# kvas7andy/unreal

Measured on AMD Instinct MI355X. Metric: env-steps/sec (whole node), UNREAL maze 84x84, higher is better.
Workload: dtype f32 (fp16x2-split MFMA operands, fp32 accumulate)

## Files before the change

### unreal_amd/csrc/pc.hip

```cpp
#include "common.h"

namespace {

constexpr int HP_LD = 36, HP_ROWS = 84;
constexpr int NPLP = 2;
constexpr int WD_ELEMS = 4 * 4 * 2 * 4 * 16 * 4;
constexpr int HP_V = (C2_POS * 8 + 255) / 256;
constexpr int DD_V = (PC_CELLS * 8 / 4 + 255) / 256;

struct PcFwdArgs {
  int N, A;
  const float* hp;
  const float* hp_absmax;
  const float* Wv; const float* bv; const float* Wa; const float* ba;
  float* qmax;
  const int* action;
  const float* target;
  const int* mask;
  float lambda, grad_scale;
  float* d_dec;
  float* ddec_absmax;
  float* loss;
};

// ... 11 lines not shown
    int id = gtid + 256 * c;
    r[c] = s4[id < C2_POS * 8 ? id : gtid];
  }
}

__device__ __forceinline__ void hp_store(float* hp, int gtid, const f32x4 (&r)[HP_V]) {
#pragma unroll
  for (int c = 0; c < HP_V; ++c) {
    int id = gtid + 256 * c;
    if (id < C2_POS * 8) *reinterpret_cast<f32x4*>(hp + (id >> 3) * HP_LD + (id & 7) * 4) = r[c];
  }
}

typedef _Float16 fh8p __attribute__((ext_vector_type(8)));
typedef _Float16 fh2p __attribute__((ext_vector_type(2)));
typedef float f32x2p __attribute__((ext_vector_type(2)));
typedef unsigned int u32x2p __attribute__((ext_vector_type(2)));

constexpr int HPP_ROW = 80;
constexpr int HPP_PLANE = HP_ROWS * HPP_ROW;
constexpr int WDP_ROW = 80;
constexpr int WDP_PLANE = 4 * 32 * WDP_ROW;

__device__ __forceinline__ void split4p(const f32x4& v, float scale, u32x2p (&pl)[NPLP]) {
  const f32x2p x01 = (f32x2p){v[0], v[1]} * scale, x23 = (f32x2p){v[2], v[3]} * scale;
  const fh2p h01 = __builtin_convertvector(x01, fh2p), h23 = __builtin_convertvector(x23, fh2p);
  const fh2p l01 = __builtin_convertvector(x01 - __builtin_convertvector(h01, f32x2p), fh2p);
  const fh2p l23 = __builtin_convertvector(x23 - __builtin_convertvector(h23, f32x2p), fh2p);
  pl[0] = (u32x2p){__builtin_bit_cast(unsigned int, h01), __builtin_bit_cast(unsigned int, h23)};
  pl[1] = (u32x2p){__builtin_bit_cast(unsigned int, l01), __builtin_bit_cast(unsigned int, l23)};
}

__device__ __forceinline__ void hp_store_planes(unsigned char* hpp, int gtid, const f32x4 (&r)[HP_V], float scale) {
#pragma unroll
  for (int c = 0; c < HP_V; ++c) {
    const int id = gtid + 256 * c;
    if (id < C2_POS * 8) {
      u32x2p pl[NPLP];
      split4p(r[c], scale, pl);
      pl[0][0] = keep_positive_visible(pl[0][0], r[c][0], r[c][1]);
      pl[0][1] = keep_positive_visible(pl[0][1], r[c][2], r[c][3]);
#pragma unroll
      for (int t = 0; t < NPLP; ++t) *reinterpret_cast<u32x2p*>(hpp + t * HPP_PLANE + (id >> 3) * HPP_ROW + (id & 7) * 8) = pl[t];
    }
  }
}

#define PC_MFMA(a, b, c) __builtin_amdgcn_mfma_f32_16x16x32_f16((a), (b), (c), 0, 0, 0)
#define PC_SPLIT_MMA(A, B, C)        \
  do {                               \
    C = PC_MFMA(A[1], B[0], C);      \
    C = PC_MFMA(A[0], B[1], C);      \
    C = PC_MFMA(A[0], B[0], C);      \
  } while (0)

__device__ __forceinline__ float pc_weight_max(const float* __restrict__ Wv, const float* __restrict__ Wa, int A, float* red) {
  if (threadIdx.x == 0) *red = 0.f;
  __syncthreads();
  float m = 0.f;
  for (int e = threadIdx.x; e < 512; e += 256) m = fmaxf(m, fabsf(Wv[e]));
  for (int e = threadIdx.x; e < 512 * A; e += 256) m = fmaxf(m, fabsf(Wa[e]));
  m = wave_max(m);
  if ((threadIdx.x & 63) == 0) atomicMax(reinterpret_cast<unsigned int*>(red), __float_as_uint(m));
  __syncthreads();
  return *red;
}

__device__ __forceinline__ void pc_fwd_weight_planes(const float* __restrict__ Wv, const float* __restrict__ Wa, int A,
                                                     unsigned char* wdp, float S_W) {
  const int CO = 1 + A;
  for (int e = threadIdx.x; e < 4 * 32 * 8; e += 256) {
    const int c4 = e & 7, n = (e >> 3) & 31, dd = e >> 8;
    f32x4 v = {0.f, 0.f, 0.f, 0.f};
    if (n < 4 * CO) {
      const int par = n / CO, co = n - par * CO;
      const int ky = (par >> 1) + 2 * (dd >> 1), kx = (par & 1) + 2 * (dd & 1);
#pragma unroll
      for (int k = 0; k < 4; ++k) v[k] = deconv_w(Wv, Wa, A, ky, kx, co, 4 * c4 + k);
    }
    u32x2p pl[NPLP];
    split4p(v, S_W, pl);
#pragma unroll
    for (int t = 0; t < NPLP; ++t) *reinterpret_cast<u32x2p*>(wdp + t * WDP_PLANE + (dd * 32 + n) * WDP_ROW + c4 * 8) = pl[t];
  }
}

__device__ __forceinline__ void pc_zero_hp_pad_rows(unsigned char* hpp) {
  for (int e = threadIdx.x; e < NPLP * 3 * HPP_ROW / 4; e += 256) {
    const int t = e / (3 * HPP_ROW / 4), w = e % (3 * HPP_ROW / 4);
    reinterpret_cast<uint32_t*>(hpp + t * HPP_PLANE + C2_POS * HPP_ROW)[w] = 0u;
  }
}

template <int COT> struct FwdLds {
  static constexpr int DS = COT | 1;
  static constexpr int DEC = NPLP * HPP_PLANE, DOUT = DEC + PC_CELLS * DS * 4, W = DOUT + PC_CELLS * COT * 4,
                       BYTES = W + NPLP * WDP_PLANE;
  static constexpr int WGS = 3 * BYTES <= 160 * 1024 ? 3 : 2;
};

template <bool TWO_NT, int DS>
__device__ __forceinline__ void deconv_packed(const unsigned char* hpp, const unsigned char* wdp, float* dec, int mt0, int i,
                                              int q, int CO, const float (&bias)[2], float unscale) {
  constexpr int NTL = TWO_NT ? 2 : 1;
  const int ntiles = (mt0 + 4 < 7) ? 2 : 1;
  f32x4 acc[2][NTL];
  int a[2], b[2];
#pragma unroll
  for (int t = 0; t < 2; ++t) {
#pragma unroll
    for (int nt = 0; nt < NTL; ++nt) acc[t][nt] = (f32x4){0.f, 0.f, 0.f, 0.f};
    const int m = min((mt0 + 4 * t) * 16 + i, 99);
    a[t] = m / 10;
    b[t] = m % 10;
  }
#pragma unroll
  for (int dd = 0; dd < 4; ++dd) {
    const int da = dd >> 1, db = dd & 1;
    fh8p bw[NTL][NPLP];
#pragma unroll
    for (int nt = 0; nt < NTL; ++nt)
#pragma unroll
      for (int pl = 0; pl < NPLP; ++pl)
        bw[nt][pl] = *reinterpret_cast<const fh8p*>(wdp + pl * WDP_PLANE + ((dd * 32 + nt * 16 + i)) * WDP_ROW + 16 * q);
#pragma unroll
    for (int t = 0; t < 2; ++t) {
      if (t < ntiles) {
        const int y = a[t] - da, x = b[t] - db;
        const int row = (y >= 0 && y < 9 && x >= 0 && x < 9) ? y * 9 + x : C2_POS;
        fh8p av[NPLP];
#pragma unroll
        for (int pl = 0; pl < NPLP; ++pl)
          av[pl] = *reinterpret_cast<const fh8p*>(hpp + pl * HPP_PLANE + row * HPP_ROW + 16 * q);
#pragma unroll
        for (int nt = 0; nt < NTL; ++nt) PC_SPLIT_MMA(av, bw[nt], acc[t][nt]);
      }
    }
  }
#pragma unroll
  for (int nt = 0; nt < NTL; ++nt) {
    const int n = nt * 16 + i;
    if (n < 4 * CO) {
      const int par = n / CO, co = n - par * CO;
#pragma unroll
      for (int t = 0; t < 2; ++t)
        if (t < ntiles) {
#pragma unroll
          for (int r = 0; r < 4; ++r) {
            const int m = (mt0 + 4 * t) * 16 + 4 * q + r;
            if (m < 100)
              dec[((2 * (m / 10) + (par >> 1)) * 20 + 2 * (m % 10) + (par & 1)) * DS + co] = acc[t][nt][r] * unscale + bias[nt];
          }
        }
    }
  }
}

template <int COT>
__global__ __launch_bounds__(256, FwdLds<COT>::WGS) void pc_deconv_fwd_kernel(PcFwdArgs p) {
  typedef FwdLds<COT> L;
  constexpr int DS = L::DS;
  __shared__ __attribute__((aligned(16))) unsigned char smem[L::BYTES];
  __shared__ float s_red;
  const int gtid = threadIdx.x;
  const int lane = threadIdx.x & 63, gw = gtid >> 6;
  const int i = lane & 15, q = lane >> 4;
  unsigned char* hpp = smem;
  float* dec = reinterpret_cast<float*>(smem + L::DEC);
  float* dout = reinterpret_cast<float*>(smem + L::DOUT);
  unsigned char* wdp = smem + L::W;
  const int A = p.A, CO = 1 + p.A;

  const float S_W = pow2_scale(pc_weight_max(p.Wv, p.Wa, A, &s_red));
  const float S_HP = pow2_scale(*p.hp_absmax);
  const float unscale = pow2_inv(S_HP) * pow2_inv(S_W);

  pc_fwd_weight_planes(p.Wv, p.Wa, A, wdp, S_W);
  pc_zero_hp_pad_rows(hpp);
  float bias[2];
#pragma unroll
  for (int nt = 0; nt < 2; ++nt) {
    const int n = nt * 16 + i;
    const int co = n % CO;
    bias[nt] = (n < 4 * CO) ? (co == 0 ? p.bv[0] : p.ba[co - 1]) : 0.f;
  }
  const bool two_nt = 4 * CO > 16;
  float loss_acc = 0.f, dd_max = 0.f;

  const int stride = gridDim.x;
  f32x4 pre[HP_V];
  {
    const int n0 = blockIdx.x;
    if (n0 < p.N) {
      hp_load(p.hp + (size_t)n0 * F2_DIM, gtid, pre);
      hp_store_planes(hpp, gtid, pre, S_HP);
    }
  }
  int prev = -1;
  for (int base = blockIdx.x; base < p.N; base += stride) {
    const int n = base;
    const bool valid = n < p.N;
// ... 67 lines not shown
      if (p.ddec_absmax) absmax_commit(p.ddec_absmax, fmaxf(fmaxf(wmx[0], wmx[1]), fmaxf(wmx[2], wmx[3])));
    }
  }
}

struct PcBwdArgs {
  int N, A;
  const float* hp;
  const float* hp_absmax;
  const float* d_dec;
  const float* ddec_absmax;
  const float* Wv; const float* Wa;
  float* d_hp;
  float* dWv; float* dbv; float* dWa; float* dba;
  float* dhp_absmax;
};

typedef short s16x4p __attribute__((ext_vector_type(4)));
typedef short s16x8p __attribute__((ext_vector_type(8)));
constexpr int DDP_ROW = 16;
constexpr int DDP_PLANE = (PC_CELLS + 4) * DDP_ROW;
constexpr int WBP_PLANE = 4 * 32 * WDP_ROW;
constexpr int BWD_GRP_BYTES = NPLP * HPP_PLANE + NPLP * DDP_PLANE + F2_DIM * 4;

__device__ __forceinline__ fh8p tr_pair_p(const unsigned char* a0, const unsigned char* a1) {
  typedef s16x4p __attribute__((address_space(3))) * lds_p;
  const s16x4p lo = __builtin_amdgcn_ds_read_tr16_b64_v4i16((lds_p)(a0));
  const s16x4p hi = __builtin_amdgcn_ds_read_tr16_b64_v4i16((lds_p)(a1));
  const s16x8p v = __builtin_shufflevector(lo, hi, 0, 1, 2, 3, 4, 5, 6, 7);
  return __builtin_bit_cast(fh8p, v);
}

__device__ __forceinline__ void split1p(float x, float scale, unsigned short (&t)[NPLP]) {
  x *= scale;
  const _Float16 h = (_Float16)x;
  const _Float16 l = (_Float16)(x - (float)h);
  t[0] = __builtin_bit_cast(unsigned short, h);
  t[1] = __builtin_bit_cast(unsigned short, l);
}

__device__ __forceinline__ void pc_bwd_weight_planes(const float* __restrict__ Wv, const float* __restrict__ Wa, int A,
                                                     unsigned char* wbp, float S_W) {
  for (int e = threadIdx.x; e < 4 * 32 * 32; e += 256) {
    const int k = e & 31, ci = (e >> 5) & 31, ky = e >> 10;
    const int kx = k >> 3, co = k & 7;
    float v = 0.f;
    if (co == 0) v = Wv[(ky * 4 + kx) * 32 + ci];
    else if (co <= A) v = Wa[((ky * 4 + kx) * A + (co - 1)) * 32 + ci];
    unsigned short t[NPLP];
    split1p(v, S_W, t);
#pragma unroll
    for (int pl = 0; pl < NPLP; ++pl)
      reinterpret_cast<unsigned short*>(wbp + pl * WBP_PLANE + (ky * 32 + ci) * WDP_ROW)[k] = t[pl];
  }
}

__device__ __forceinline__ void pc_stage_dd(unsigned char* ddp, int gtid, const float (&dd)[2][8], float S_DD, float (&adbk)[8]) {
#pragma unroll
  for (int h = 0; h < 2; ++h) {
    const int pos = gtid + 256 * h;
    if (pos < PC_CELLS) {
      u32x2p lo[NPLP], hi[NPLP];
      split4p((f32x4){dd[h][0], dd[h][1], dd[h][2], dd[h][3]}, S_DD, lo);
      split4p((f32x4){dd[h][4], dd[h][5], dd[h][6], dd[h][7]}, S_DD, hi);
#pragma unroll
      for (int pl = 0; pl < NPLP; ++pl) {
        typedef unsigned int u32x4p __attribute__((ext_vector_type(4)));
        *reinterpret_cast<u32x4p*>(ddp + pl * DDP_PLANE + pos * DDP_ROW) = (u32x4p){lo[pl][0], lo[pl][1], hi[pl][0], hi[pl][1]};
      }
#pragma unroll
      for (int k = 0; k < 8; ++k) adbk[k] += dd[h][k];
    }
  }
}

__device__ __forceinline__ void pc_dgrad_frame(const unsigned char* hpp, const unsigned char* ddp, const unsigned char* wbp,
                                               float* dhs, int gw, int i, int q, float un_dgrad) {
  const int nt = gw & 1;
  f32x4 acc[3];
  int abase[3];
#pragma unroll
  for (int jj = 0; jj < 3; ++jj) {
    acc[jj] = (f32x4){0.f, 0.f, 0.f, 0.f};
    const int pos = min(((gw >> 1) + 2 * jj) * 16 + i, C2_POS - 1);
    abase[jj] = ((2 * (pos / 9)) * 20 + 2 * (pos % 9) + q) * DDP_ROW;
  }
#pragma unroll
  for (int ky = 0; ky < 4; ++ky) {
    fh8p bw[NPLP];
#pragma unroll
    for (int pl = 0; pl < NPLP; ++pl)
      bw[pl] = *reinterpret_cast<const fh8p*>(wbp + pl * WBP_PLANE + (ky * 32 + nt * 16 + i) * WDP_ROW + 16 * q);
#pragma unroll
    for (int jj = 0; jj < 3; ++jj) {
      fh8p av[NPLP];
#pragma unroll
      for (int pl = 0; pl < NPLP; ++pl)
        av[pl] = *reinterpret_cast<const fh8p*>(ddp + pl * DDP_PLANE + abase[jj] + ky * 20 * DDP_ROW);
      PC_SPLIT_MMA(av, bw, acc[jj]);
    }
  }
#pragma unroll
  for (int jj = 0; jj < 3; ++jj)
#pragma unroll
    for (int r = 0; r < 4; ++r) {
      const int pos = ((gw >> 1) + 2 * jj) * 16 + 4 * q + r;
      if (pos < C2_POS) {
        const int ci = nt * 16 + i;
        const unsigned short h0 = reinterpret_cast<const unsigned short*>(hpp + pos * HPP_ROW)[ci];
        dhs[pos * 32 + ci] = (h0 != 0 && !(h0 & 0x8000)) ? acc[jj][r] * un_dgrad : 0.f;
      }
    }
}

__device__ __forceinline__ void pc_wgrad_frame(const unsigned char* hpp, const unsigned char* ddp, int gw, int i, int q,
                                               f32x4 (&aw)[2][2]) {
  const int qq = i >> 2, pp = i & 3;
#pragma unroll 1
  for (int ks = 0; ks < 3; ++ks) {
    const int p0 = 32 * ks + 8 * q + qq, p1 = p0 + 4;
    const unsigned char* b0 = hpp + min(p0, C2_POS) * HPP_ROW + 8 * pp;
    const unsigned char* b1 = hpp + min(p1, C2_POS) * HPP_ROW + 8 * pp;
    fh8p bf[2][NPLP];
#pragma unroll
    for (int t = 0; t < 2; ++t)
#pragma unroll
      for (int pl = 0; pl < NPLP; ++pl) bf[t][pl] = tr_pair_p(b0 + pl * HPP_PLANE + 32 * t, b1 + pl * HPP_PLANE + 32 * t);
    const int r0 = p0 < C2_POS ? (2 * (p0 / 9) + gw) * 20 + 2 * (p0 % 9) : PC_CELLS;
    const int r1 = p1 < C2_POS ? (2 * (p1 / 9) + gw) * 20 + 2 * (p1 % 9) : PC_CELLS;
#pragma unroll
    for (int kxh = 0; kxh < 2; ++kxh) {
      fh8p af[NPLP];
#pragma unroll
      for (int pl = 0; pl < NPLP; ++pl)
        af[pl] = tr_pair_p(ddp + pl * DDP_PLANE + (r0 + 2 * kxh) * DDP_ROW + 8 * pp,
                           ddp + pl * DDP_PLANE + (r1 + 2 * kxh) * DDP_ROW + 8 * pp);
      PC_SPLIT_MMA(af, bf[0], aw[kxh][0]);
      PC_SPLIT_MMA(af, bf[1], aw[kxh][1]);
    }
  }
}

__device__ __forceinline__ float pc_drain_dhp(const float* dhs, float* __restrict__ dst_frame, int gtid, float dhp_max) {
  f32x4* dst = reinterpret_cast<f32x4*>(dst_frame);
  for (int id = gtid; id < F2_DIM / 4; id += 256) {
    const f32x4 v = reinterpret_cast<const f32x4*>(dhs)[id];
    dst[id] = v;
    dhp_max = fmaxf(fmaxf(dhp_max, fmaxf(fabsf(v[0]), fabsf(v[1]))), fmaxf(fabsf(v[2]), fabsf(v[3])));
  }
  return dhp_max;
}

__device__ __forceinline__ void pc_commit_grads(const f32x4 (&aw)[2][2], float un_wgrad, const float (&adbk)[8], float dhp_max,
                                                int A, float* dWv, float* dWa, float* dbv, float* dba, float* dhp_absmax,
                                                float* red, int gw, int lane, int i, int q) {
  const int gtid = threadIdx.x, CO = 1 + A;
#pragma unroll
  for (int kxh = 0; kxh < 2; ++kxh)
#pragma unroll
    for (int t = 0; t < 2; ++t)
#pragma unroll
      for (int r = 0; r < 4; ++r) {
        int row = 4 * q + r;
        int kx = 2 * kxh + (row >> 3), co = row & 7, ci = t * 16 + i;
        float v = aw[kxh][t][r] * un_wgrad;
        if (co == 0) atomicAdd(dWv + (gw * 4 + kx) * 32 + ci, v);
        else if (co <= A) atomicAdd(dWa + ((gw * 4 + kx) * A + (co - 1)) * 32 + ci, v);
      }
  float* wsum = red;
  float* wmx = red + 32;
#pragma unroll
  for (int k = 0; k < 8; ++k) {
    const float v = wave_sum(adbk[k]);
    if (lane == 0) wsum[gw * 8 + k] = v;
  }
  dhp_max = wave_max(dhp_max);
  if (lane == 0) wmx[gw] = dhp_max;
  __syncthreads();
  if (gtid < CO) {
    const float v = ((wsum[gtid] + wsum[8 + gtid]) + wsum[16 + gtid]) + wsum[24 + gtid];
    if (gtid == 0) atomicAdd(dbv, v);
    else atomicAdd(dba + (gtid - 1), v);
  }
  if (gw == 0) absmax_commit(dhp_absmax, fmaxf(fmaxf(wmx[0], wmx[1]), fmaxf(wmx[2], wmx[3])));
}

__global__ __launch_bounds__(256, 2) void pc_deconv_bwd_kernel(PcBwdArgs p) {
  __shared__ __attribute__((aligned(16))) unsigned char smem[BWD_GRP_BYTES + NPLP * WBP_PLANE];
  __shared__ float s_red[36];
  static_assert(2 * (BWD_GRP_BYTES + NPLP * WBP_PLANE + 144) <= 160 * 1024, "two workgroups must fit one CU's LDS");
  const int gtid = threadIdx.x;
  const int lane = threadIdx.x & 63, gw = gtid >> 6;
  const int i = lane & 15, q = lane >> 4;
  unsigned char* hpp = smem;
  unsigned char* ddp = hpp + NPLP * HPP_PLANE;
  float* dhs = reinterpret_cast<float*>(ddp + NPLP * DDP_PLANE);
  unsigned char* wbp = smem + BWD_GRP_BYTES;
  const int A = p.A, CO = 1 + p.A;

  const float S_W = pow2_scale(pc_weight_max(p.Wv, p.Wa, A, s_red));
  const float S_HP = pow2_scale(*p.hp_absmax), S_DD = pow2_scale(*p.ddec_absmax);
  const float un_dgrad = pow2_inv(S_DD) * pow2_inv(S_W);
  const float un_wgrad = pow2_inv(S_DD) * pow2_inv(S_HP);

  pc_bwd_weight_planes(p.Wv, p.Wa, A, wbp, S_W);
  pc_zero_hp_pad_rows(hpp);
  for (int e = gtid; e < NPLP * DDP_PLANE / 4; e += 256) reinterpret_cast<uint32_t*>(ddp)[e] = 0u;

  f32x4 aw[2][2];
#pragma unroll
  for (int a = 0; a < 2; ++a)
#pragma unroll
    for (int b = 0; b < 2; ++b) aw[a][b] = (f32x4){0.f, 0.f, 0.f, 0.f};
  float adbk[8];
#pragma unroll
  for (int k = 0; k < 8; ++k) adbk[k] = 0.f;
  float dhp_max = 0.f;

  const int stride = gridDim.x;
  f32x4 pre_hp[HP_V];
  float pre_dd[2][8];
  auto load_dd = [&](int frame) {
    const float* src = p.d_dec + (size_t)frame * PC_CELLS * CO;
#pragma unroll
    for (int h = 0; h < 2; ++h) {
      const int pos = min(gtid + 256 * h, PC_CELLS - 1);
#pragma unroll
      for (int co = 0; co < 8; ++co) pre_dd[h][co] = (co < CO) ? src[pos * CO + co] : 0.f;
    }
// ... 6 lines not shown
      hp_load(p.hp + (size_t)n0 * F2_DIM, gtid, pre_hp);
      hp_store_planes(hpp, gtid, pre_hp, S_HP);
      load_dd(n0);
      pc_stage_dd(ddp, gtid, pre_dd, S_DD, adbk);
    }
  }
  for (int n = blockIdx.x; n < p.N; n += stride) {
    const int nn = n + stride;
    const bool has_next = nn < p.N;
    __syncthreads();
    if (has_next) {
      hp_load(p.hp + (size_t)nn * F2_DIM, gtid, pre_hp);
      load_dd(nn);
    }
    pc_dgrad_frame(hpp, ddp, wbp, dhs, gw, i, q, un_dgrad);
    pc_wgrad_frame(hpp, ddp, gw, i, q, aw);
    __syncthreads();
    dhp_max = pc_drain_dhp(dhs, p.d_hp + (size_t)n * F2_DIM, gtid, dhp_max);
    if (has_next) {
      hp_store_planes(hpp, gtid, pre_hp, S_HP);
      pc_stage_dd(ddp, gtid, pre_dd, S_DD, adbk);
    }
  }
  pc_commit_grads(aw, un_wgrad, adbk, dhp_max, A, p.dWv, p.dWa, p.dbv, p.dba, p.dhp_absmax, s_red, gw, lane, i, q);
}

struct PcTrainArgs {
  int N, A;
  const float* hp; const float* hp_absmax;
  const float* Wv; const float* bv; const float* Wa; const float* ba;
  const int* action; const float* target; const int* mask;
  float lambda, grad_scale;
  float* loss;
  float* d_hp; float* dhp_absmax;
  float* dWv; float* dbv; float* dWa; float* dba;
  float* d_dec;
};

template <int COT> struct TrainLds {
  static constexpr int DS = COT | 1;
  static constexpr int UNI = PC_CELLS * DS * 4 > F2_DIM * 4 ? PC_CELLS * DS * 4 : F2_DIM * 4;
  static constexpr int DDP = NPLP * HPP_PLANE, U = DDP + NPLP * DDP_PLANE, WF = U + UNI, WB = WF + NPLP * WDP_PLANE,
                       RED = WB + NPLP * WBP_PLANE, BYTES = RED + 192;
  static constexpr int WGS = 2 * BYTES <= 160 * 1024 ? 2 : 1;
};

template <int COT>
__global__ __launch_bounds__(256, TrainLds<COT>::WGS) void pc_deconv_train_kernel(PcTrainArgs p) {
  typedef TrainLds<COT> L;
  constexpr int DS = L::DS;
  __shared__ __attribute__((aligned(16))) unsigned char smem[L::BYTES];
  const int gtid = threadIdx.x;
  const int lane = threadIdx.x & 63, gw = gtid >> 6;
  const int i = lane & 15, q = lane >> 4;
  unsigned char* hpp = smem;
  unsigned char* ddp = smem + L::DDP;
  float* uni = reinterpret_cast<float*>(smem + L::U);
  unsigned char* wdp = smem + L::WF;
  unsigned char* wbp = smem + L::WB;
  float* red = reinterpret_cast<float*>(smem + L::RED);
  const int A = p.A, CO = 1 + p.A;

  const float S_W = pow2_scale(pc_weight_max(p.Wv, p.Wa, A, red));
  const float S_HP = pow2_scale(*p.hp_absmax);
  const float un_fwd = pow2_inv(S_HP) * pow2_inv(S_W);
  pc_fwd_weight_planes(p.Wv, p.Wa, A, wdp, S_W);
  pc_bwd_weight_planes(p.Wv, p.Wa, A, wbp, S_W);
  pc_zero_hp_pad_rows(hpp);
  for (int e = gtid; e < NPLP * DDP_PLANE / 4; e += 256) reinterpret_cast<uint32_t*>(ddp)[e] = 0u;
  float bias[2];
#pragma unroll
  for (int nt = 0; nt < 2; ++nt) {
    const int n = nt * 16 + i;
    const int co = n % CO;
    bias[nt] = (n < 4 * CO) ? (co == 0 ? p.bv[0] : p.ba[co - 1]) : 0.f;
  }
  const bool two_nt = 4 * CO > 16;

  f32x4 aw[2][2];
#pragma unroll
  for (int a = 0; a < 2; ++a)
#pragma unroll
    for (int b = 0; b < 2; ++b) aw[a][b] = (f32x4){0.f, 0.f, 0.f, 0.f};
  float adbk[8];
#pragma unroll
  for (int k = 0; k < 8; ++k) adbk[k] = 0.f;
  float dhp_max = 0.f, loss_acc = 0.f;

  const int stride = gridDim.x;
  f32x4 pre[HP_V];
  __syncthreads();
  if (blockIdx.x < p.N) {
    hp_load(p.hp + (size_t)blockIdx.x * F2_DIM, gtid, pre);
    hp_store_planes(hpp, gtid, pre, S_HP);
  }
  for (int n = blockIdx.x; n < p.N; n += stride) {
    const int nn = n + stride;
    const bool has_next = nn < p.N;
    __syncthreads();
    if (has_next) hp_load(p.hp + (size_t)nn * F2_DIM, gtid, pre);
    const float tg[2] = {p.target[(size_t)n * PC_CELLS + gtid], p.target[(size_t)n * PC_CELLS + min(gtid + 256, PC_CELLS - 1)]};
    const int act = p.action[n];
    const bool on = p.mask[n] != 0;
    if (two_nt) deconv_packed<true, DS>(hpp, wdp, uni, gw, i, q, CO, bias, un_fwd);
    else deconv_packed<false, DS>(hpp, wdp, uni, gw, i, q, CO, bias, un_fwd);
    __syncthreads();
    float dd[2][8];
    float fmx = 0.f;
#pragma unroll
    for (int pi = 0; pi < 2; ++pi) {
#pragma unroll
      for (int k = 0; k < 8; ++k) dd[pi][k] = 0.f;
      const int pos = gtid + 256 * pi;
      if (pos < PC_CELLS) {
        const float* d = uni + pos * DS;
        const float vpre = d[0];
        const float V = fmaxf(vpre, 0.f);
        float apre[COT - 1], mean = 0.f, aact = 0.f;
#pragma unroll
        for (int k = 0; k < COT - 1; ++k) {
          apre[k] = k < A ? d[1 + k] : 0.f;
          const float ad = fmaxf(apre[k], 0.f);
          mean += ad;
          aact = (k == act) ? ad : aact;
        }
        mean /= (float)A;
        const float qa = V + aact - mean;
        const float diff = tg[pi] - qa;
        const float dq = on ? -p.lambda * diff * p.grad_scale : 0.f;
        if (on) loss_acc += 0.5f * p.lambda * diff * diff;
        fmx = fmaxf(fmx, fabsf(dq));
        dd[pi][0] = vpre > 0.f ? dq : 0.f;
#pragma unroll
        for (int k = 0; k < COT - 1; ++k)
          dd[pi][1 + k] = (k < A && apre[k] > 0.f) ? dq * (((k == act) ? 1.f : 0.f) - 1.f / (float)A) : 0.f;
        if (p.d_dec) {
          float* o = p.d_dec + ((size_t)n * PC_CELLS + pos) * CO;
#pragma unroll
          for (int k = 0; k < COT; ++k)
            if (k < CO) o[k] = dd[pi][k];
        }
      }
    }
    fmx = wave_max(fmx);
    if (lane == 0) red[40 + gw] = fmx;
    __syncthreads();
    const float S_DD = pow2_scale(fmaxf(fmaxf(red[40], red[41]), fmaxf(red[42], red[43])));
    const float inv_dd = pow2_inv(S_DD);
    pc_stage_dd(ddp, gtid, dd, S_DD, adbk);
    __syncthreads();
    pc_dgrad_frame(hpp, ddp, wbp, uni, gw, i, q, inv_dd * pow2_inv(S_W));
    {
      f32x4 awf[2][2];
#pragma unroll
      for (int a = 0; a < 2; ++a)
#pragma unroll
        for (int b = 0; b < 2; ++b) awf[a][b] = (f32x4){0.f, 0.f, 0.f, 0.f};
      pc_wgrad_frame(hpp, ddp, gw, i, q, awf);
#pragma unroll
      for (int a = 0; a < 2; ++a)
#pragma unroll
        for (int b = 0; b < 2; ++b) aw[a][b] += awf[a][b] * inv_dd;
    }
    __syncthreads();
    dhp_max = pc_drain_dhp(uni, p.d_hp + (size_t)n * F2_DIM, gtid, dhp_max);
    if (has_next) hp_store_planes(hpp, gtid, pre, S_HP);
  }
  __syncthreads();
  loss_acc = wave_sum(loss_acc);
  if (lane == 0) red[44 + gw] = loss_acc;
  pc_commit_grads(aw, pow2_inv(S_HP), adbk, dhp_max, A, p.dWv, p.dWa, p.dbv, p.dba, p.dhp_absmax, red, gw, lane, i, q);
  if (gtid == 0) atomicAdd(p.loss, (((red[44] + red[45]) + red[46]) + red[47]) * p.grad_scale);
}

constexpr int WIDE_CO = UNREAL_MAX_ACTIONS + 1;
constexpr int WIDE_HS_LD = 33;
constexpr int WIDE_HS_BYTES = 82 * WIDE_HS_LD * 4;
constexpr int WIDE_WT_LD = 32 * WIDE_CO;
constexpr int WIDE_WS_BYTES = 16 * WIDE_WT_LD * 4;
constexpr int WIDE_DD_BYTES = PC_CELLS * WIDE_CO * 4;
constexpr int WIDE_WG_ENTRIES = (16 * WIDE_CO + 7) / 8;
constexpr int WIDE_FWD_BYTES = WIDE_HS_BYTES + WIDE_WS_BYTES;
constexpr int WIDE_TRAIN_BYTES = WIDE_FWD_BYTES + WIDE_DD_BYTES;
static_assert(3 * (WIDE_FWD_BYTES + 64) <= 160 * 1024, "three wide forward workgroups must fit one CU's LDS");
static_assert(2 * (WIDE_TRAIN_BYTES + 192) <= 160 * 1024, "two wide training workgroups must fit one CU's LDS");

__device__ __forceinline__ void wide_stage_weights(const float* __restrict__ Wv, const float* __restrict__ Wa, int A,
                                                   float* ws) {
  for (int e = threadIdx.x; e < 16 * 32 * WIDE_CO; e += 256) {
    const int co = e % WIDE_CO, ci = (e / WIDE_CO) & 31, tap = e / (32 * WIDE_CO);
    float v = 0.f;
    if (co == 0) v = Wv[tap * 32 + ci];
    else if (co <= A) v = Wa[(tap * A + (co - 1)) * 32 + ci];
    ws[e] = v;
  }
// ... 342 lines not shown
    hipLaunchKernelGGL(pc_deconv_bwd_wide_kernel, dim3(blocks), dim3(256), 0, (hipStream_t)stream, p);
    return unreal_launch_status();
  }
  hipLaunchKernelGGL(pc_deconv_bwd_kernel, dim3(blocks), dim3(256), 0, (hipStream_t)stream, p);
  return unreal_launch_status();
}

int unreal_pc_deconv_train(int N, int A, const float* hp, const float* hp_absmax, const float* Wv, const float* bv,
                           const float* Wa, const float* ba, const int* action, const float* target, const int* mask,
                           float lambda, float grad_scale, float* loss, float* d_hp, float* dhp_absmax, float* dWv, float* dbv,
                           float* dWa, float* dba, float* d_dec, void* stream) {
  if (N <= 0 || A <= 0 || A > UNREAL_MAX_ACTIONS || !hp || !hp_absmax || !Wv || !bv || !Wa || !ba || !action || !target ||
      !mask || !loss ||
      !d_hp || !dWv || !dbv || !dWa || !dba)
    return UNREAL_EINVAL;
  if ((((uintptr_t)hp) | ((uintptr_t)d_hp)) & 15) return UNREAL_EINVAL;
  PcTrainArgs p{N, A, hp, hp_absmax, Wv, bv, Wa, ba, action, target, mask, lambda, grad_scale, loss, d_hp, dhp_absmax,
                dWv, dbv, dWa, dba, d_dec};
  hipStream_t st = (hipStream_t)stream;
  if (A > 7) {
    hipLaunchKernelGGL(pc_deconv_train_wide_kernel, dim3(min(N, 256 * 2)), dim3(256), 0, st, p);
    return unreal_launch_status();
  }
#define PC_TRAIN(COT) \
  hipLaunchKernelGGL(pc_deconv_train_kernel<COT>, dim3(min(N, 256 * TrainLds<COT>::WGS)), dim3(256), 0, st, p)
  switch (1 + A) {
    case 4: PC_TRAIN(4); break;
    case 5: PC_TRAIN(5); break;
    case 7: PC_TRAIN(7); break;
    default: PC_TRAIN(8); break;
  }
#undef PC_TRAIN
  return unreal_launch_status();
}

}
```

Before: 3.758 million.

## Share weight planes across frame groups per workgroup and swizzle LDS layout

The pixel-control train kernel now runs several 256-thread frame groups inside one larger workgroup. The groups share a single copy of the forward and backward weight planes, so each workgroup builds those planes once instead of once per 256-thread block. Shared-memory frame planes switch from padded rows to an XOR-swizzled 64-byte row layout, which is meant to avoid bank conflicts while using less LDS. Per-group gradient sums are reduced through LDS before a single commit, which cuts global atomics. The costs are a larger workgroup with more barriers across groups and a changed prefetch position for the next frame.

```diff
diff --git a/unreal_amd/csrc/pc.hip b/unreal_amd/csrc/pc.hip
--- a/unreal_amd/csrc/pc.hip
+++ b/unreal_amd/csrc/pc.hip
@@ -57,6 +57,26 @@
 constexpr int WDP_ROW = 80;
 constexpr int WDP_PLANE = 4 * 32 * WDP_ROW;
 
+struct PcPadded {
+  static constexpr int HP_ROW = HPP_ROW, W_ROW = WDP_ROW, DD_LD = 20;
+  static __device__ __forceinline__ int row64(int row, int b, int) { return row * 80 + b; }
+  static __device__ __forceinline__ int row64(int row, int b) { return row * 80 + b; }
+};
+struct PcSwizzled {
+  static constexpr int HP_ROW = 64, W_ROW = 64, DD_LD = 25;
+  static __device__ __forceinline__ int row64(int row, int b, int x) { return row * 64 + (b ^ (((-x) & 3) << 4)); }
+  static __device__ __forceinline__ int row64(int row, int b) { return (row * 64 + (((-(row >> 2)) & 3) << 4)) ^ b; }
+};
+template <class LY> struct PcPlanes {
+  static constexpr int HP_PLANE = HP_ROWS * LY::HP_ROW, W_PLANE = 4 * 32 * LY::W_ROW;
+  static constexpr int DD_ZERO = 20 * LY::DD_LD;
+  static constexpr int DD_PLANE = (DD_ZERO + 4) * 16;
+  static __device__ __forceinline__ int dd(int pos) {
+    if constexpr (LY::DD_LD == 20) return pos * 16;
+    else return ((pos / 20) * LY::DD_LD + pos % 20) * 16;
+  }
+};
+
 __device__ __forceinline__ void split4p(const f32x4& v, float scale, u32x2p (&pl)[NPLP]) {
   const f32x2p x01 = (f32x2p){v[0], v[1]} * scale, x23 = (f32x2p){v[2], v[3]} * scale;
   const fh2p h01 = __builtin_convertvector(x01, fh2p), h23 = __builtin_convertvector(x23, fh2p);
@@ -66,6 +86,7 @@
   pl[1] = (u32x2p){__builtin_bit_cast(unsigned int, l01), __builtin_bit_cast(unsigned int, l23)};
 }
 
+template <class LY = PcPadded>
 __device__ __forceinline__ void hp_store_planes(unsigned char* hpp, int gtid, const f32x4 (&r)[HP_V], float scale) {
 #pragma unroll
   for (int c = 0; c < HP_V; ++c) {
@@ -76,7 +97,8 @@
       pl[0][0] = keep_positive_visible(pl[0][0], r[c][0], r[c][1]);
       pl[0][1] = keep_positive_visible(pl[0][1], r[c][2], r[c][3]);
 #pragma unroll
-      for (int t = 0; t < NPLP; ++t) *reinterpret_cast<u32x2p*>(hpp + t * HPP_PLANE + (id >> 3) * HPP_ROW + (id & 7) * 8) = pl[t];
+      for (int t = 0; t < NPLP; ++t)
+        *reinterpret_cast<u32x2p*>(hpp + t * PcPlanes<LY>::HP_PLANE + LY::row64(id >> 3, (id & 7) * 8, (gtid >> 5) & 3)) = pl[t];
     }
   }
 }
@@ -89,22 +111,24 @@
     C = PC_MFMA(A[0], B[0], C);      \
   } while (0)
 
-__device__ __forceinline__ float pc_weight_max(const float* __restrict__ Wv, const float* __restrict__ Wa, int A, float* red) {
+__device__ __forceinline__ float pc_weight_max(const float* __restrict__ Wv, const float* __restrict__ Wa, int A, float* red,
+                                               int nthr) {
   if (threadIdx.x == 0) *red = 0.f;
   __syncthreads();
   float m = 0.f;
-  for (int e = threadIdx.x; e < 512; e += 256) m = fmaxf(m, fabsf(Wv[e]));
-  for (int e = threadIdx.x; e < 512 * A; e += 256) m = fmaxf(m, fabsf(Wa[e]));
+  for (int e = threadIdx.x; e < 512; e += nthr) m = fmaxf(m, fabsf(Wv[e]));
+  for (int e = threadIdx.x; e < 512 * A; e += nthr) m = fmaxf(m, fabsf(Wa[e]));
   m = wave_max(m);
   if ((threadIdx.x & 63) == 0) atomicMax(reinterpret_cast<unsigned int*>(red), __float_as_uint(m));
   __syncthreads();
   return *red;
 }
 
+template <class LY = PcPadded>
 __device__ __forceinline__ void pc_fwd_weight_planes(const float* __restrict__ Wv, const float* __restrict__ Wa, int A,
-                                                     unsigned char* wdp, float S_W) {
+                                                     unsigned char* wdp, float S_W, int nthr) {
   const int CO = 1 + A;
-  for (int e = threadIdx.x; e < 4 * 32 * 8; e += 256) {
+  for (int e = threadIdx.x; e < 4 * 32 * 8; e += nthr) {
     const int c4 = e & 7, n = (e >> 3) & 31, dd = e >> 8;
     f32x4 v = {0.f, 0.f, 0.f, 0.f};
     if (n < 4 * CO) {
@@ -116,14 +140,15 @@
     u32x2p pl[NPLP];
     split4p(v, S_W, pl);
 #pragma unroll
-    for (int t = 0; t < NPLP; ++t) *reinterpret_cast<u32x2p*>(wdp + t * WDP_PLANE + (dd * 32 + n) * WDP_ROW + c4 * 8) = pl[t];
-  }
-}
-
-__device__ __forceinline__ void pc_zero_hp_pad_rows(unsigned char* hpp) {
-  for (int e = threadIdx.x; e < NPLP * 3 * HPP_ROW / 4; e += 256) {
-    const int t = e / (3 * HPP_ROW / 4), w = e % (3 * HPP_ROW / 4);
-    reinterpret_cast<uint32_t*>(hpp + t * HPP_PLANE + C2_POS * HPP_ROW)[w] = 0u;
+    for (int t = 0; t < NPLP; ++t) *reinterpret_cast<u32x2p*>(wdp + t * PcPlanes<LY>::W_PLANE + LY::row64(dd * 32 + n, c4 * 8)) = pl[t];
+  }
+}
+
+template <class LY = PcPadded>
+__device__ __forceinline__ void pc_zero_hp_pad_rows(unsigned char* hpp, int gtid) {
+  for (int e = gtid; e < NPLP * 3 * LY::HP_ROW / 4; e += 256) {
+    const int t = e / (3 * LY::HP_ROW / 4), w = e % (3 * LY::HP_ROW / 4);
+    reinterpret_cast<uint32_t*>(hpp + t * PcPlanes<LY>::HP_PLANE + C2_POS * LY::HP_ROW)[w] = 0u;
   }
 }
 
@@ -134,7 +159,7 @@
   static constexpr int WGS = 3 * BYTES <= 160 * 1024 ? 3 : 2;
 };
 
-template <bool TWO_NT, int DS>
+template <bool TWO_NT, int DS, class LY = PcPadded>
 __device__ __forceinline__ void deconv_packed(const unsigned char* hpp, const unsigned char* wdp, float* dec, int mt0, int i,
                                               int q, int CO, const float (&bias)[2], float unscale) {
   constexpr int NTL = TWO_NT ? 2 : 1;
@@ -157,7 +182,8 @@
     for (int nt = 0; nt < NTL; ++nt)
 #pragma unroll
       for (int pl = 0; pl < NPLP; ++pl)
-        bw[nt][pl] = *reinterpret_cast<const fh8p*>(wdp + pl * WDP_PLANE + ((dd * 32 + nt * 16 + i)) * WDP_ROW + 16 * q);
+        bw[nt][pl] = *reinterpret_cast<const fh8p*>(wdp + pl * PcPlanes<LY>::W_PLANE +
+                                                    LY::row64(dd * 32 + nt * 16 + i, 16 * q, (i >> 2) & 3));
 #pragma unroll
     for (int t = 0; t < 2; ++t) {
       if (t < ntiles) {
@@ -166,7 +192,7 @@
         fh8p av[NPLP];
 #pragma unroll
         for (int pl = 0; pl < NPLP; ++pl)
-          av[pl] = *reinterpret_cast<const fh8p*>(hpp + pl * HPP_PLANE + row * HPP_ROW + 16 * q);
+          av[pl] = *reinterpret_cast<const fh8p*>(hpp + pl * PcPlanes<LY>::HP_PLANE + LY::row64(row, 16 * q));
 #pragma unroll
         for (int nt = 0; nt < NTL; ++nt) PC_SPLIT_MMA(av, bw[nt], acc[t][nt]);
       }
@@ -206,12 +232,12 @@
   unsigned char* wdp = smem + L::W;
   const int A = p.A, CO = 1 + p.A;
 
-  const float S_W = pow2_scale(pc_weight_max(p.Wv, p.Wa, A, &s_red));
+  const float S_W = pow2_scale(pc_weight_max(p.Wv, p.Wa, A, &s_red, 256));
   const float S_HP = pow2_scale(*p.hp_absmax);
   const float unscale = pow2_inv(S_HP) * pow2_inv(S_W);
 
-  pc_fwd_weight_planes(p.Wv, p.Wa, A, wdp, S_W);
-  pc_zero_hp_pad_rows(hpp);
+  pc_fwd_weight_planes(p.Wv, p.Wa, A, wdp, S_W, 256);
+  pc_zero_hp_pad_rows(hpp, gtid);
   float bias[2];
 #pragma unroll
   for (int nt = 0; nt < 2; ++nt) {
@@ -325,6 +351,9 @@
 constexpr int DDP_PLANE = (PC_CELLS + 4) * DDP_ROW;
 constexpr int WBP_PLANE = 4 * 32 * WDP_ROW;
 constexpr int BWD_GRP_BYTES = NPLP * HPP_PLANE + NPLP * DDP_PLANE + F2_DIM * 4;
+static_assert(PcPlanes<PcPadded>::HP_PLANE == HPP_PLANE && PcPlanes<PcPadded>::W_PLANE == WDP_PLANE &&
+              PcPlanes<PcPadded>::W_PLANE == WBP_PLANE && PcPlanes<PcPadded>::DD_PLANE == DDP_PLANE,
+              "the padded layout is the one these constants describe");
 
 __device__ __forceinline__ fh8p tr_pair_p(const unsigned char* a0, const unsigned char* a1) {
   typedef s16x4p __attribute__((address_space(3))) * lds_p;
@@ -342,9 +371,10 @@
   t[1] = __builtin_bit_cast(unsigned short, l);
 }
 
+template <class LY = PcPadded>
 __device__ __forceinline__ void pc_bwd_weight_planes(const float* __restrict__ Wv, const float* __restrict__ Wa, int A,
-                                                     unsigned char* wbp, float S_W) {
-  for (int e = threadIdx.x; e < 4 * 32 * 32; e += 256) {
+                                                     unsigned char* wbp, float S_W, int nthr) {
+  for (int e = threadIdx.x; e < 4 * 32 * 32; e += nthr) {
     const int k = e & 31, ci = (e >> 5) & 31, ky = e >> 10;
     const int kx = k >> 3, co = k & 7;
     float v = 0.f;
@@ -354,10 +384,11 @@
     split1p(v, S_W, t);
 #pragma unroll
     for (int pl = 0; pl < NPLP; ++pl)
-      reinterpret_cast<unsigned short*>(wbp + pl * WBP_PLANE + (ky * 32 + ci) * WDP_ROW)[k] = t[pl];
-  }
-}
-
+      *reinterpret_cast<unsigned short*>(wbp + pl * PcPlanes<LY>::W_PLANE + LY::row64(ky * 32 + ci, 2 * k)) = t[pl];
+  }
+}
+
+template <class LY = PcPadded>
 __device__ __forceinline__ void pc_stage_dd(unsigned char* ddp, int gtid, const float (&dd)[2][8], float S_DD, float (&adbk)[8]) {
 #pragma unroll
   for (int h = 0; h < 2; ++h) {
@@ -369,7 +400,8 @@
 #pragma unroll
       for (int pl = 0; pl < NPLP; ++pl) {
         typedef unsigned int u32x4p __attribute__((ext_vector_type(4)));
-        *reinterpret_cast<u32x4p*>(ddp + pl * DDP_PLANE + pos * DDP_ROW) = (u32x4p){lo[pl][0], lo[pl][1], hi[pl][0], hi[pl][1]};
+        *reinterpret_cast<u32x4p*>(ddp + pl * PcPlanes<LY>::DD_PLANE + PcPlanes<LY>::dd(pos)) =
+            (u32x4p){lo[pl][0], lo[pl][1], hi[pl][0], hi[pl][1]};
       }
 #pragma unroll
       for (int k = 0; k < 8; ++k) adbk[k] += dd[h][k];
@@ -377,8 +409,10 @@
   }
 }
 
+template <class LY = PcPadded>
 __device__ __forceinline__ void pc_dgrad_frame(const unsigned char* hpp, const unsigned char* ddp, const unsigned char* wbp,
                                                float* dhs, int gw, int i, int q, float un_dgrad) {
+  typedef PcPlanes<LY> P;
   const int nt = gw & 1;
   f32x4 acc[3];
   int abase[3];
@@ -386,20 +420,20 @@
   for (int jj = 0; jj < 3; ++jj) {
     acc[jj] = (f32x4){0.f, 0.f, 0.f, 0.f};
     const int pos = min(((gw >> 1) + 2 * jj) * 16 + i, C2_POS - 1);
-    abase[jj] = ((2 * (pos / 9)) * 20 + 2 * (pos % 9) + q) * DDP_ROW;
+    abase[jj] = ((2 * (pos / 9)) * LY::DD_LD + 2 * (pos % 9) + q) * DDP_ROW;
   }
 #pragma unroll
   for (int ky = 0; ky < 4; ++ky) {
     fh8p bw[NPLP];
 #pragma unroll
     for (int pl = 0; pl < NPLP; ++pl)
-      bw[pl] = *reinterpret_cast<const fh8p*>(wbp + pl * WBP_PLANE + (ky * 32 + nt * 16 + i) * WDP_ROW + 16 * q);
+      bw[pl] = *reinterpret_cast<const fh8p*>(wbp + pl * P::W_PLANE + LY::row64(ky * 32 + nt * 16 + i, 16 * q, (i >> 2) & 3));
 #pragma unroll
     for (int jj = 0; jj < 3; ++jj) {
       fh8p av[NPLP];
 #pragma unroll
       for (int pl = 0; pl < NPLP; ++pl)
-        av[pl] = *reinterpret_cast<const fh8p*>(ddp + pl * DDP_PLANE + abase[jj] + ky * 20 * DDP_ROW);
+        av[pl] = *reinterpret_cast<const fh8p*>(ddp + pl * P::DD_PLANE + abase[jj] + ky * LY::DD_LD * DDP_ROW);
       PC_SPLIT_MMA(av, bw, acc[jj]);
     }
   }
@@ -410,34 +444,37 @@
       const int pos = ((gw >> 1) + 2 * jj) * 16 + 4 * q + r;
       if (pos < C2_POS) {
         const int ci = nt * 16 + i;
-        const unsigned short h0 = reinterpret_cast<const unsigned short*>(hpp + pos * HPP_ROW)[ci];
+        const unsigned short h0 = *reinterpret_cast<const unsigned short*>(hpp + LY::row64(pos, 2 * ci, q));
         dhs[pos * 32 + ci] = (h0 != 0 && !(h0 & 0x8000)) ? acc[jj][r] * un_dgrad : 0.f;
       }
     }
 }
 
+template <class LY = PcPadded>
 __device__ __forceinline__ void pc_wgrad_frame(const unsigned char* hpp, const unsigned char* ddp, int gw, int i, int q,
                                                f32x4 (&aw)[2][2]) {
+  typedef PcPlanes<LY> P;
   const int qq = i >> 2, pp = i & 3;
 #pragma unroll 1
   for (int ks = 0; ks < 3; ++ks) {
     const int p0 = 32 * ks + 8 * q + qq, p1 = p0 + 4;
-    const unsigned char* b0 = hpp + min(p0, C2_POS) * HPP_ROW + 8 * pp;
-    const unsigned char* b1 = hpp + min(p1, C2_POS) * HPP_ROW + 8 * pp;
     fh8p bf[2][NPLP];
 #pragma unroll
-    for (int t = 0; t < 2; ++t)
-#pragma unroll
-      for (int pl = 0; pl < NPLP; ++pl) bf[t][pl] = tr_pair_p(b0 + pl * HPP_PLANE + 32 * t, b1 + pl * HPP_PLANE + 32 * t);
-    const int r0 = p0 < C2_POS ? (2 * (p0 / 9) + gw) * 20 + 2 * (p0 % 9) : PC_CELLS;
-    const int r1 = p1 < C2_POS ? (2 * (p1 / 9) + gw) * 20 + 2 * (p1 % 9) : PC_CELLS;
+    for (int t = 0; t < 2; ++t) {
+      const unsigned char* b0 = hpp + LY::row64(min(p0, C2_POS), 8 * pp + 32 * t, (2 * q) & 3);
+      const unsigned char* b1 = hpp + LY::row64(min(p1, C2_POS), 8 * pp + 32 * t, (2 * q + 1) & 3);
+#pragma unroll
+      for (int pl = 0; pl < NPLP; ++pl) bf[t][pl] = tr_pair_p(b0 + pl * P::HP_PLANE, b1 + pl * P::HP_PLANE);
+    }
+    const int r0 = p0 < C2_POS ? (2 * (p0 / 9) + gw) * LY::DD_LD + 2 * (p0 % 9) : P::DD_ZERO;
+    const int r1 = p1 < C2_POS ? (2 * (p1 / 9) + gw) * LY::DD_LD + 2 * (p1 % 9) : P::DD_ZERO;
 #pragma unroll
     for (int kxh = 0; kxh < 2; ++kxh) {
       fh8p af[NPLP];
 #pragma unroll
       for (int pl = 0; pl < NPLP; ++pl)
-        af[pl] = tr_pair_p(ddp + pl * DDP_PLANE + (r0 + 2 * kxh) * DDP_ROW + 8 * pp,
-                           ddp + pl * DDP_PLANE + (r1 + 2 * kxh) * DDP_ROW + 8 * pp);
+        af[pl] = tr_pair_p(ddp + pl * P::DD_PLANE + (r0 + 2 * kxh) * DDP_ROW + 8 * pp,
+                           ddp + pl * P::DD_PLANE + (r1 + 2 * kxh) * DDP_ROW + 8 * pp);
       PC_SPLIT_MMA(af, bf[0], aw[kxh][0]);
       PC_SPLIT_MMA(af, bf[1], aw[kxh][1]);
     }
@@ -456,36 +493,38 @@
 
 __device__ __forceinline__ void pc_commit_grads(const f32x4 (&aw)[2][2], float un_wgrad, const float (&adbk)[8], float dhp_max,
                                                 int A, float* dWv, float* dWa, float* dbv, float* dba, float* dhp_absmax,
-                                                float* red, int gw, int lane, int i, int q) {
-  const int gtid = threadIdx.x, CO = 1 + A;
-#pragma unroll
-  for (int kxh = 0; kxh < 2; ++kxh)
-#pragma unroll
-    for (int t = 0; t < 2; ++t)
-#pragma unroll
-      for (int r = 0; r < 4; ++r) {
-        int row = 4 * q + r;
-        int kx = 2 * kxh + (row >> 3), co = row & 7, ci = t * 16 + i;
-        float v = aw[kxh][t][r] * un_wgrad;
-        if (co == 0) atomicAdd(dWv + (gw * 4 + kx) * 32 + ci, v);
-        else if (co <= A) atomicAdd(dWa + ((gw * 4 + kx) * A + (co - 1)) * 32 + ci, v);
-      }
+                                                float* red, bool commits, int gtid, int gw, int lane, int i, int q) {
+  const int CO = 1 + A;
   float* wsum = red;
   float* wmx = red + 32;
-#pragma unroll
-  for (int k = 0; k < 8; ++k) {
-    const float v = wave_sum(adbk[k]);
-    if (lane == 0) wsum[gw * 8 + k] = v;
-  }
-  dhp_max = wave_max(dhp_max);
-  if (lane == 0) wmx[gw] = dhp_max;
+  if (commits) {
+#pragma unroll
+    for (int kxh = 0; kxh < 2; ++kxh)
+#pragma unroll
+      for (int t = 0; t < 2; ++t)
+#pragma unroll
+        for (int r = 0; r < 4; ++r) {
+          int row = 4 * q + r;
+          int kx = 2 * kxh + (row >> 3), co = row & 7, ci = t * 16 + i;
+          float v = aw[kxh][t][r] * un_wgrad;
+          if (co == 0) atomicAdd(dWv + (gw * 4 + kx) * 32 + ci, v);
+          else if (co <= A) atomicAdd(dWa + ((gw * 4 + kx) * A + (co - 1)) * 32 + ci, v);
+        }
+#pragma unroll
+    for (int k = 0; k < 8; ++k) {
+      const float v = wave_sum(adbk[k]);
+      if (lane == 0) wsum[gw * 8 + k] = v;
+    }
+    dhp_max = wave_max(dhp_max);
+    if (lane == 0) wmx[gw] = dhp_max;
+  }
   __syncthreads();
-  if (gtid < CO) {
+  if (commits && gtid < CO) {
     const float v = ((wsum[gtid] + wsum[8 + gtid]) + wsum[16 + gtid]) + wsum[24 + gtid];
     if (gtid == 0) atomicAdd(dbv, v);
     else atomicAdd(dba + (gtid - 1), v);
   }
-  if (gw == 0) absmax_commit(dhp_absmax, fmaxf(fmaxf(wmx[0], wmx[1]), fmaxf(wmx[2], wmx[3])));
+  if (commits && gw == 0) absmax_commit(dhp_absmax, fmaxf(fmaxf(wmx[0], wmx[1]), fmaxf(wmx[2], wmx[3])));
 }
 
 __global__ __launch_bounds__(256, 2) void pc_deconv_bwd_kernel(PcBwdArgs p) {
@@ -501,13 +540,13 @@
   unsigned char* wbp = smem + BWD_GRP_BYTES;
   const int A = p.A, CO = 1 + p.A;
 
-  const float S_W = pow2_scale(pc_weight_max(p.Wv, p.Wa, A, s_red));
+  const float S_W = pow2_scale(pc_weight_max(p.Wv, p.Wa, A, s_red, 256));
   const float S_HP = pow2_scale(*p.hp_absmax), S_DD = pow2_scale(*p.ddec_absmax);
   const float un_dgrad = pow2_inv(S_DD) * pow2_inv(S_W);
   const float un_wgrad = pow2_inv(S_DD) * pow2_inv(S_HP);
 
-  pc_bwd_weight_planes(p.Wv, p.Wa, A, wbp, S_W);
-  pc_zero_hp_pad_rows(hpp);
+  pc_bwd_weight_planes(p.Wv, p.Wa, A, wbp, S_W, 256);
+  pc_zero_hp_pad_rows(hpp, gtid);
   for (int e = gtid; e < NPLP * DDP_PLANE / 4; e += 256) reinterpret_cast<uint32_t*>(ddp)[e] = 0u;
 
   f32x4 aw[2][2];
@@ -560,7 +599,7 @@
       pc_stage_dd(ddp, gtid, pre_dd, S_DD, adbk);
     }
   }
-  pc_commit_grads(aw, un_wgrad, adbk, dhp_max, A, p.dWv, p.dWa, p.dbv, p.dba, p.dhp_absmax, s_red, gw, lane, i, q);
+  pc_commit_grads(aw, un_wgrad, adbk, dhp_max, A, p.dWv, p.dWa, p.dbv, p.dba, p.dhp_absmax, s_red, true, gtid, gw, lane, i, q);
 }
 
 struct PcTrainArgs {
@@ -578,34 +617,42 @@
 template <int COT> struct TrainLds {
   static constexpr int DS = COT | 1;
   static constexpr int UNI = PC_CELLS * DS * 4 > F2_DIM * 4 ? PC_CELLS * DS * 4 : F2_DIM * 4;
-  static constexpr int DDP = NPLP * HPP_PLANE, U = DDP + NPLP * DDP_PLANE, WF = U + UNI, WB = WF + NPLP * WDP_PLANE,
-                       RED = WB + NPLP * WBP_PLANE, BYTES = RED + 192;
-  static constexpr int WGS = 2 * BYTES <= 160 * 1024 ? 2 : 1;
+  typedef PcSwizzled LY;
+  typedef PcPlanes<LY> P;
+  static constexpr int DDP = NPLP * P::HP_PLANE, U = DDP + NPLP * P::DD_PLANE, SET = U + UNI;
+  static constexpr int WEIGHTS = 2 * NPLP * P::W_PLANE, RED_BYTES = 256;
+  static constexpr int GROUPS = 3 * SET + WEIGHTS + RED_BYTES <= 160 * 1024 ? 3 : 2;
+  static constexpr int WF = GROUPS * SET, WB = WF + NPLP * P::W_PLANE, RED = WB + NPLP * P::W_PLANE, BYTES = RED + RED_BYTES;
+  static constexpr int STASH = 26;
+  static_assert(BYTES <= 160 * 1024, "the frame sets and one weight image must fit a workgroup's LDS");
+  static_assert(SET % 16 == 0 && STASH * 256 * 4 <= SET, "frame sets are 16-byte aligned and hold a group's final sums");
 };
 
 template <int COT>
-__global__ __launch_bounds__(256, TrainLds<COT>::WGS) void pc_deconv_train_kernel(PcTrainArgs p) {
+__global__ __launch_bounds__(256 * TrainLds<COT>::GROUPS, 1) void pc_deconv_train_kernel(PcTrainArgs p) {
   typedef TrainLds<COT> L;
-  constexpr int DS = L::DS;
+  typedef typename L::LY LY;
+  constexpr int DS = L::DS, NG = L::GROUPS, NTHR = 256 * NG;
   __shared__ __attribute__((aligned(16))) unsigned char smem[L::BYTES];
-  const int gtid = threadIdx.x;
-  const int lane = threadIdx.x & 63, gw = gtid >> 6;
+  const int g = threadIdx.x / 256, gtid = threadIdx.x % 256;
+  const int lane = threadIdx.x & 63, gw = (threadIdx.x >> 6) & 3;
   const int i = lane & 15, q = lane >> 4;
-  unsigned char* hpp = smem;
-  unsigned char* ddp = smem + L::DDP;
-  float* uni = reinterpret_cast<float*>(smem + L::U);
+  unsigned char* hpp = smem + g * L::SET;
+  unsigned char* ddp = hpp + L::DDP;
+  float* uni = reinterpret_cast<float*>(hpp + L::U);
   unsigned char* wdp = smem + L::WF;
   unsigned char* wbp = smem + L::WB;
   float* red = reinterpret_cast<float*>(smem + L::RED);
-  const int A = p.A, CO = 1 + p.A;
-
-  const float S_W = pow2_scale(pc_weight_max(p.Wv, p.Wa, A, red));
+  float* gmx = red + 40 + 4 * g;
+  const int A = COT < 8 ? COT - 1 : p.A, CO = 1 + A;
+
+  const float S_W = pow2_scale(pc_weight_max(p.Wv, p.Wa, A, red, NTHR));
   const float S_HP = pow2_scale(*p.hp_absmax);
   const float un_fwd = pow2_inv(S_HP) * pow2_inv(S_W);
-  pc_fwd_weight_planes(p.Wv, p.Wa, A, wdp, S_W);
-  pc_bwd_weight_planes(p.Wv, p.Wa, A, wbp, S_W);
-  pc_zero_hp_pad_rows(hpp);
-  for (int e = gtid; e < NPLP * DDP_PLANE / 4; e += 256) reinterpret_cast<uint32_t*>(ddp)[e] = 0u;
+  pc_fwd_weight_planes<LY>(p.Wv, p.Wa, A, wdp, S_W, NTHR);
+  pc_bwd_weight_planes<LY>(p.Wv, p.Wa, A, wbp, S_W, NTHR);
+  pc_zero_hp_pad_rows<LY>(hpp, gtid);
+  for (int e = gtid; e < NPLP * L::P::DD_PLANE / 4; e += 256) reinterpret_cast<uint32_t*>(ddp)[e] = 0u;
   float bias[2];
 #pragma unroll
   for (int nt = 0; nt < 2; ++nt) {
@@ -625,23 +672,33 @@
   for (int k = 0; k < 8; ++k) adbk[k] = 0.f;
   float dhp_max = 0.f, loss_acc = 0.f;
 
-  const int stride = gridDim.x;
+  const int stride = gridDim.x * NG;
+  const int rounds = (p.N + stride - 1) / stride;
   f32x4 pre[HP_V];
   __syncthreads();
-  if (blockIdx.x < p.N) {
-    hp_load(p.hp + (size_t)blockIdx.x * F2_DIM, gtid, pre);
-    hp_store_planes(hpp, gtid, pre, S_HP);
-  }
-  for (int n = blockIdx.x; n < p.N; n += stride) {
+  int n = blockIdx.x * NG + g;
+  if (n < p.N) {
+    hp_load(p.hp + (size_t)n * F2_DIM, gtid, pre);
+    hp_store_planes<LY>(hpp, gtid, pre, S_HP);
+  }
+  for (int r = 0; r < rounds; ++r, n += stride) {
+    const bool live = n < p.N;
     const int nn = n + stride;
     const bool has_next = nn < p.N;
     __syncthreads();
-    if (has_next) hp_load(p.hp + (size_t)nn * F2_DIM, gtid, pre);
-    const float tg[2] = {p.target[(size_t)n * PC_CELLS + gtid], p.target[(size_t)n * PC_CELLS + min(gtid + 256, PC_CELLS - 1)]};
-    const int act = p.action[n];
-    const bool on = p.mask[n] != 0;
-    if (two_nt) deconv_packed<true, DS>(hpp, wdp, uni, gw, i, q, CO, bias, un_fwd);
-    else deconv_packed<false, DS>(hpp, wdp, uni, gw, i, q, CO, bias, un_fwd);
+    float tg[2] = {0.f, 0.f};
+    int act = 0;
+    bool on = false;
+    if (live) {
+      tg[0] = p.target[(size_t)n * PC_CELLS + gtid];
+      tg[1] = p.target[(size_t)n * PC_CELLS + min(gtid + 256, PC_CELLS - 1)];
+      act = p.action[n];
+      on = p.mask[n] != 0;
+      int qf = q, fi = i;
+      asm volatile("" : "+v"(qf), "+v"(fi));
+      if (two_nt) deconv_packed<true, DS, LY>(hpp, wdp, uni, gw, fi, qf, CO, bias, un_fwd);
+      else deconv_packed<false, DS, LY>(hpp, wdp, uni, gw, fi, qf, CO, bias, un_fwd);
+    }
     __syncthreads();
     float dd[2][8];
     float fmx = 0.f;
@@ -650,7 +707,7 @@
 #pragma unroll
       for (int k = 0; k < 8; ++k) dd[pi][k] = 0.f;
       const int pos = gtid + 256 * pi;
-      if (pos < PC_CELLS) {
+      if (live && pos < PC_CELLS) {
         const float* d = uni + pos * DS;
         const float vpre = d[0];
         const float V = fmaxf(vpre, 0.f);
@@ -681,34 +738,68 @@
       }
     }
     fmx = wave_max(fmx);
-    if (lane == 0) red[40 + gw] = fmx;
-    __syncthreads();
-    const float S_DD = pow2_scale(fmaxf(fmaxf(red[40], red[41]), fmaxf(red[42], red[43])));
+    if (lane == 0) gmx[gw] = fmx;
+    __syncthreads();
+    const float S_DD = pow2_scale(fmaxf(fmaxf(gmx[0], gmx[1]), fmaxf(gmx[2], gmx[3])));
     const float inv_dd = pow2_inv(S_DD);
-    pc_stage_dd(ddp, gtid, dd, S_DD, adbk);
-    __syncthreads();
-    pc_dgrad_frame(hpp, ddp, wbp, uni, gw, i, q, inv_dd * pow2_inv(S_W));
-    {
+    if (live) pc_stage_dd<LY>(ddp, gtid, dd, S_DD, adbk);
+    __syncthreads();
+    if (has_next) hp_load(p.hp + (size_t)nn * F2_DIM, gtid, pre);
+    if (live) {
+      int qb = q;
+      asm volatile("" : "+v"(qb));
+      pc_dgrad_frame<LY>(hpp, ddp, wbp, uni, gw, i, qb, inv_dd * pow2_inv(S_W));
       f32x4 awf[2][2];
 #pragma unroll
       for (int a = 0; a < 2; ++a)
 #pragma unroll
         for (int b = 0; b < 2; ++b) awf[a][b] = (f32x4){0.f, 0.f, 0.f, 0.f};
-      pc_wgrad_frame(hpp, ddp, gw, i, q, awf);
+      pc_wgrad_frame<LY>(hpp, ddp, gw, i, q, awf);
 #pragma unroll
       for (int a = 0; a < 2; ++a)
 #pragma unroll
         for (int b = 0; b < 2; ++b) aw[a][b] += awf[a][b] * inv_dd;
     }
     __syncthreads();
-    dhp_max = pc_drain_dhp(uni, p.d_hp + (size_t)n * F2_DIM, gtid, dhp_max);
-    if (has_next) hp_store_planes(hpp, gtid, pre, S_HP);
+    if (live) dhp_max = pc_drain_dhp(uni, p.d_hp + (size_t)n * F2_DIM, gtid, dhp_max);
+    if (has_next) hp_store_planes<LY>(hpp, gtid, pre, S_HP);
   }
   __syncthreads();
-  loss_acc = wave_sum(loss_acc);
-  if (lane == 0) red[44 + gw] = loss_acc;
-  pc_commit_grads(aw, pow2_inv(S_HP), adbk, dhp_max, A, p.dWv, p.dWa, p.dbv, p.dba, p.dhp_absmax, red, gw, lane, i, q);
-  if (gtid == 0) atomicAdd(p.loss, (((red[44] + red[45]) + red[46]) + red[47]) * p.grad_scale);
+  if (g > 0) {
+    float* st = reinterpret_cast<float*>(hpp) + gtid;
+#pragma unroll
+    for (int a = 0; a < 2; ++a)
+#pragma unroll
+      for (int b = 0; b < 2; ++b)
+#pragma unroll
+        for (int k = 0; k < 4; ++k) st[((a * 2 + b) * 4 + k) * 256] = aw[a][b][k];
+#pragma unroll
+    for (int k = 0; k < 8; ++k) st[(16 + k) * 256] = adbk[k];
+    st[24 * 256] = loss_acc;
+    st[25 * 256] = dhp_max;
+  }
+  __syncthreads();
+  if (g == 0) {
+#pragma unroll
+    for (int gg = 1; gg < NG; ++gg) {
+      const float* st = reinterpret_cast<const float*>(smem + gg * L::SET) + gtid;
+#pragma unroll
+      for (int a = 0; a < 2; ++a)
+#pragma unroll
+        for (int b = 0; b < 2; ++b)
+#pragma unroll
+          for (int k = 0; k < 4; ++k) aw[a][b][k] += st[((a * 2 + b) * 4 + k) * 256];
+#pragma unroll
+      for (int k = 0; k < 8; ++k) adbk[k] += st[(16 + k) * 256];
+      loss_acc += st[24 * 256];
+      dhp_max = fmaxf(dhp_max, st[25 * 256]);
+    }
+    loss_acc = wave_sum(loss_acc);
+    if (lane == 0) red[36 + gw] = loss_acc;
+  }
+  pc_commit_grads(aw, pow2_inv(S_HP), adbk, dhp_max, A, p.dWv, p.dWa, p.dbv, p.dba, p.dhp_absmax, red, g == 0, gtid, gw, lane,
+                  i, q);
+  if (threadIdx.x == 0) atomicAdd(p.loss, (((red[36] + red[37]) + red[38]) + red[39]) * p.grad_scale);
 }
 
 constexpr int WIDE_CO = UNREAL_MAX_ACTIONS + 1;
@@ -1097,8 +1188,9 @@
     hipLaunchKernelGGL(pc_deconv_train_wide_kernel, dim3(min(N, 256 * 2)), dim3(256), 0, st, p);
     return unreal_launch_status();
   }
-#define PC_TRAIN(COT) \
-  hipLaunchKernelGGL(pc_deconv_train_kernel<COT>, dim3(min(N, 256 * TrainLds<COT>::WGS)), dim3(256), 0, st, p)
+#define PC_TRAIN(COT)                                                                                                     \
+  hipLaunchKernelGGL(pc_deconv_train_kernel<COT>, dim3(min((N + TrainLds<COT>::GROUPS - 1) / TrainLds<COT>::GROUPS, 256)), \
+                     dim3(256 * TrainLds<COT>::GROUPS), 0, st, p)
   switch (1 + A) {
     case 4: PC_TRAIN(4); break;
     case 5: PC_TRAIN(5); break;
```

New measurement: 3.781 million, median of 6. Within noise of the previous version (+0.6%).
